# muzishen/RCDMs

Hardware: AMD Instinct MI355X
Metric: story-frames/sec (stage-2 UNet, 50-step DDIM, 512^2) (higher is better)
Workload: dtype f16; 1 GPU; PororoSV stage-2, 512x512, 50-step DDIM, CFG 2.0, batch=1 story x 5 frames per GPU, ctx 85x768, random-init 1276.9M-param UNet3D; stories_per_gpu=1, latent=64, ddim_steps=50, parallelism=story-replicas x1

## Files before the change

rcdms_amd/csrc/rowff.hip:

```cpp
#include "common.h"
#include "pp_sync.h"
#include <type_traits>

#ifndef RCDM_FF_ABLATE
#define RCDM_FF_ABLATE 0
#endif

namespace {

enum { TAIL_FF = 0, TAIL_N1 = 1, TAIL_FFP = 2, TAIL_N3 = 3, TAIL_ATT = 4 };

struct RowArgs {
  const f16* a_in;
  const f16* res;
  f16* tok;
  f16* out;
  const f16* wstream;
  const float* a_bias;
  const float* ln_g;
  const float* ln_b;
  const float* pe;
  const float* b1p;
  const float* b2;
  const f16* z_res;
  const float* z_bias;
  const float* gn_stat;
  const float* gn_g;
  const float* gn_b;
  int M, lda, ldr, ldt, ldo, ldz;
  int rows_per_frame, frames;
  int gn_G, gn_rows;
  float eps;
  float att_scale;
};

template <int C, int NW, int R, int PD, bool HAS_A, bool A_RES, bool LN_PE, int TAIL>
__global__ __launch_bounds__(NW * 64) void row_chain_kernel(const RowArgs p) {
  constexpr int NK = C / 32;
  constexpr int NOF = C / 16;
  constexpr int CHF = 2 * NK;
  constexpr int CHB = CHF * 1024;
  constexpr int NG = C / 8;
  constexpr int NCH_A = HAS_A ? NK : 0;
  constexpr bool IS_FF = TAIL == TAIL_FF || TAIL == TAIL_FFP;
  constexpr bool FM = TAIL == TAIL_ATT;
  constexpr int NCH_T = IS_FF ? 3 * NG + (TAIL == TAIL_FFP ? NK : 0) : (FM ? 3 : TAIL) * NK;
  constexpr int NCH = NCH_A + NCH_T;
  constexpr int NT = NW * 64;
  constexpr int PPW = CHF / NW;
  static_assert(CHF % NW == 0, "chunk fragments must divide over the waves");
  static_assert(NOF == CHF && CHF % PD == 0 && CHF >= 20 && NOF % 2 == 0, "chunk geometry");
  constexpr int PAR0 = R * CHB;
  constexpr int RS = 2 * C + 16;
  static_assert(!IS_FF || NW * 16 * RS <= R * CHB, "epilogue staging exceeds the ring");
  constexpr int XOFF = PAR0 + 3 * C * 4, XW = (NK / 2) * 1024;
  static_assert(!FM || (HAS_A && NW == 10 && (5 * C + NW * 2 * C) * 4 <= NW * XW), "frame-major chain geometry");
  extern __shared__ __attribute__((aligned(16))) char smem[];

  const int t = threadIdx.x, lane = t & 63;
  const int wave = __builtin_amdgcn_readfirstlane(t >> 6);
  const int l15 = lane & 15, kg = lane >> 4;
  int row0_ = blockIdx.x * (NW * 16) + wave * 16, fm_gps = 1, fm_ngrp = 0;
  bool fm_live = true;
  const int fm_f = wave % 5;
  if constexpr (FM) {
    fm_gps = p.rows_per_frame >> 4;
    fm_ngrp = (p.M / (5 * p.rows_per_frame)) * fm_gps;
    const int grp = 2 * blockIdx.x + wave / 5;
    fm_live = grp < fm_ngrp;
    const int g2 = fm_live ? grp : 0, b = g2 / fm_gps;
    row0_ = (b * 5 + fm_f) * p.rows_per_frame + 16 * (g2 - b * fm_gps);
  }
  const int row0 = row0_;
  const int row = row0 + l15;
  const bool live = FM ? fm_live : row < p.M;
  const int oG = HAS_A ? C : 0, oB = oG + C, oPE = oB + C, oT = oPE + (LN_PE ? p.frames * C : 0);
  const int oZ = oT + (IS_FF ? 8 * C : 0);
  const int oGN = oZ + (TAIL == TAIL_FFP ? 2 * C : 0);
  const int npar = oGN;

  const __amdgpu_buffer_rsrc_t rsrcW =
      __builtin_amdgcn_make_buffer_rsrc((void*)p.wstream, 0, (unsigned)NCH * CHB, 0x00020000);
  int dma_voff = lane * 16;
  auto issue_chunk = [&](int c, int slot) __attribute__((always_inline)) {
#pragma unroll
    for (int i = 0; i < PPW; ++i) {
      const int piece = wave * PPW + i;
      const unsigned voff = c < NCH ? (unsigned)dma_voff : 0x80000000u;
      __builtin_amdgcn_raw_ptr_buffer_load_lds(rsrcW, (__attribute__((address_space(3))) void*)(smem + slot * CHB + piece * 1024),
                                               16, voff, c < NCH ? c * CHB + piece * 1024 : 0, 0, 0);
    }
  };

  f16x8 xr[NK];
  f16x8 tk[NK];
  auto ld16 = [](const f16* q) __attribute__((always_inline)) -> f16x8 { Pack16 t; t.u = *(const uint4*)q; return t.h; };
  auto st16 = [](f16* q, f16x8 v) __attribute__((always_inline)) { Pack16 t; t.h = v; *(uint4*)q = t.u; };
  {
    const f16* xp = p.a_in + (size_t)(live ? row : 0) * p.lda + 8 * kg;
#pragma unroll
    for (int s = 0; s < NK; ++s) xr[s] = ld16(xp + 32 * s);
    if (HAS_A && A_RES) {
      const f16* rp = p.res + (size_t)(live ? row : 0) * p.ldr + 8 * kg;
#pragma unroll
      for (int s = 0; s < NK; ++s) tk[s] = ld16(rp + 32 * s);
    } else {
#pragma unroll
      for (int s = 0; s < NK; ++s)
#pragma unroll
        for (int j = 0; j < 8; ++j) tk[s][j] = (f16)0.f;
    }
  }
  constexpr int NB4_MAX = ((HAS_A ? C : 0) + 2 * C + (LN_PE ? 8 * C : 0) + (IS_FF ? 8 * C : 0) + (TAIL == TAIL_FFP ? 2 * C : 0)) / 4;
  constexpr int NB4_PER = (NB4_MAX + NT - 1) / NT;
  f32x4 bq[NB4_PER];
#pragma unroll
  for (int i = 0; i < NB4_PER; ++i) {
    const int idx = min(i * NT + t, npar / 4 - 1) * 4;
    const float* src;
    if (HAS_A && idx < oG) src = p.a_bias + idx;
    else if (idx < oB) src = p.ln_g + (idx - oG);
    else if (idx < oPE) src = p.ln_b + (idx - oB);
    else if (LN_PE && idx < oT) src = p.pe + (idx - oPE);
    else if (idx < oZ) src = p.b1p + (idx - oT);
    else if (idx < oZ + C) src = p.b2 + (idx - oZ);
    else src = p.z_bias + (idx - oZ - C);
    bq[i] = *(const f32x4*)src;
  }
  float gn_sc = 0.f, gn_sh = 0.f;
  float fm_sc[FM ? 5 : 1], fm_sh[FM ? 5 : 1];
  constexpr bool CAN_GN = HAS_A && !A_RES;
  static_assert(NT == 2 * C, "one thread per (sample slot, channel)");
  if constexpr (FM && CAN_GN) {
    if (p.gn_stat) {
      const int j0 = t >= C ? 1 : 0, ch = t - j0 * C;
      const float ga = p.gn_g[ch], be = p.gn_b[ch];
#pragma unroll
      for (int i = 0; i < 5; ++i) {
        const int j = 2 * i + j0;
        const int smp = (min(2 * (int)blockIdx.x + j / 5, fm_ngrp - 1) / fm_gps) * 5 + j % 5;
        const float* st = p.gn_stat + ((size_t)smp * p.gn_G + ch / (C / p.gn_G)) * 2;
        const float mean = st[0], rstd = st[1];
        fm_sc[i] = rstd * ga;
        fm_sh[i] = __builtin_fmaf(-(mean * rstd), ga, be);
      }
// ... 71 lines not shown
  auto run_chunk = [&](auto&& mfma_i, auto&& slice_i, auto&& post_sync) __attribute__((always_inline)) {
    wait_vm<(R - 3) * PPW>();
    if (!(RCDM_FF_ABLATE & 8)) tick_barrier();
    if (!(RCDM_FF_ABLATE & 1)) issue_chunk(c + R - 1, cslot == 0 ? R - 1 : cslot - 1);
    post_sync();
    const char* sb = smem + cslot * CHB + lane16;
    const char* sn = smem + (cslot == R - 1 ? 0 : cslot + 1) * CHB + lane16;
    __builtin_amdgcn_sched_barrier(0);
#pragma unroll
    for (int i = 0; i < CHF; ++i) {
      const f16x8 cur = fr[i % PD];
      mfma_i(i, cur);
      fr[i % PD] = rd(i + PD < CHF ? sb + (i + PD) * 1024 : sn + (i + PD - CHF) * 1024);
      slice_i(i);
      __builtin_amdgcn_sched_barrier(0);
    }
    ++c;
    cslot = cslot == R - 1 ? 0 : cslot + 1;
  };
  auto nothing = [&](int) __attribute__((always_inline)) {};
  auto no_stores = [&]() __attribute__((always_inline)) {};
  const f32x4 z4 = {0.f, 0.f, 0.f, 0.f};

  if constexpr (HAS_A) {
#pragma unroll
    for (int h = 0; h < 2; ++h) {
      f32x4 acc[NOF / 2];
#pragma unroll
      for (int cc = 0; cc < NK / 2; ++cc)
        run_chunk([&](int i, f16x8 w) __attribute__((always_inline)) {
          const int s = 2 * cc + i / (NOF / 2), fi = i % (NOF / 2);
          acc[fi] = mm(w, xr[s], s == 0 ? z4 : acc[fi]);
        }, nothing, no_stores);
#pragma unroll
      for (int fi = 0; fi < NOF / 2; ++fi) {
        const int i = h * (NOF / 2) + fi, s = i >> 1, sub = i & 1;
        const f32x4 b = *(const f32x4*)(par + 32 * s + 8 * kg + 4 * sub);
#pragma unroll
        for (int e = 0; e < 4; ++e) tk[s][4 * sub + e] = (f16)(acc[fi][e] + b[e] + (float)tk[s][4 * sub + e]);
      }
    }
  }
  if (HAS_A && live) {
    f16* tp = p.tok + (size_t)row * p.ldt + 8 * kg;
#pragma unroll
    for (int s = 0; s < NK; ++s) st16(tp + 32 * s, tk[s]);
  }

  {
    f16x8 (&src)[NK] = HAS_A ? tk : xr;
    float s = 0.f;
#pragma unroll
    for (int k = 0; k < NK; ++k)
#pragma unroll
      for (int j = 0; j < 8; ++j) s += (float)src[k][j];
    s += __shfl_xor(s, 16, 64);
    s += __shfl_xor(s, 32, 64);
    const float mean = s * (1.0f / C);
    float q = 0.f;
#pragma unroll
    for (int k = 0; k < NK; ++k)
#pragma unroll
      for (int j = 0; j < 8; ++j) {
        const float d = (float)src[k][j] - mean;
        q += d * d;
      }
    q += __shfl_xor(q, 16, 64);
    q += __shfl_xor(q, 32, 64);
    const float rstd = rsqrtf(q * (1.0f / C) + p.eps);
    const float* pep = !LN_PE ? par : FM ? par + oPE + fm_f * C : par + oPE + (((live ? row : 0) / p.rows_per_frame) % p.frames) * C;
#pragma unroll
    for (int k = 0; k < NK; ++k) {
      const int ch = 32 * k + 8 * kg;
      const f32x4 g0 = *(const f32x4*)(par + oG + ch), g1 = *(const f32x4*)(par + oG + ch + 4);
      f32x4 b0 = *(const f32x4*)(par + oB + ch), b1 = *(const f32x4*)(par + oB + ch + 4);
      if (LN_PE) {
        b0 += *(const f32x4*)(pep + ch);
        b1 += *(const f32x4*)(pep + ch + 4);
      }
      f16x8 y;
#pragma unroll
      for (int j = 0; j < 4; ++j) {
        y[j] = (f16)(((float)src[k][j] - mean) * rstd * g0[j] + b0[j]);
        y[4 + j] = (f16)(((float)src[k][4 + j] - mean) * rstd * g1[j] + b1[j]);
      }
      xr[k] = y;
    }
  }

  auto gemm_groups = [&](auto ngrp_c, auto zadd_c) __attribute__((always_inline)) {
    constexpr int NGRP = decltype(ngrp_c)::value;
    constexpr bool ZADD = decltype(zadd_c)::value;
    f16x8 pend[NOF / 4], zr[ZADD ? NOF / 4 : 1];
    int pend_col = 0;
    auto store_pend = [&]() __attribute__((always_inline)) {
      if (live) {
        f16* op = p.out + (size_t)row * p.ldo + pend_col + 8 * kg;
#pragma unroll
        for (int m = 0; m < NOF / 4; ++m) st16(op + 32 * m, pend[m]);
      }
    };
    for (int grp = 0; grp < NGRP; ++grp) {
      f32x4 acc[NOF / 2];
#pragma unroll
      for (int cc = 0; cc < NK / 2; ++cc) {
        auto mf = [&](int i, f16x8 w) __attribute__((always_inline)) {
          const int s = 2 * cc + i / (NOF / 2), fi = i % (NOF / 2);
          acc[fi] = mm(w, xr[s], s == 0 ? z4 : acc[fi]);
        };
        if (cc == 0)
          run_chunk(mf, nothing, [&]() __attribute__((always_inline)) {
// ... 17 lines not shown
            pend[m][e] = (f16)((float)(f16)(acc[2 * m][e] + b0[e]) + (float)zr[m][e]);
            pend[m][4 + e] = (f16)((float)(f16)(acc[2 * m + 1][e] + b1[e]) + (float)zr[m][4 + e]);
          }
        } else {
#pragma unroll
          for (int e = 0; e < 4; ++e) {
            pend[m][e] = (f16)acc[2 * m][e];
            pend[m][4 + e] = (f16)acc[2 * m + 1][e];
          }
        }
      }
      pend_col = grp * (C / 2);
    }
    wait_lgkm0();
    wait_vm<0>();
    store_pend();
  };

  if constexpr (FM) {
    constexpr int HG = NK / 2;
    char* const X = smem + XOFF;
    const int kgq = lane16 >> 8, xme = wave * XW + lane16, xgrp = (wave / 5) * 5 * XW + lane16;
    const bool c1 = kgq == 0, c2 = kgq <= 1, c3 = kgq <= 2;
    f16x8 qh[HG], pend[HG], oh[HG];
    f32x4 acc[NOF / 2];
    float sc[4][5], o8[8];
    auto round_to = [&](f16x8 (&dst)[HG]) __attribute__((always_inline)) {
#pragma unroll
      for (int m = 0; m < HG; ++m)
#pragma unroll
        for (int e = 0; e < 4; ++e) {
          dst[m][e] = (f16)acc[2 * m][e];
          dst[m][4 + e] = (f16)acc[2 * m + 1][e];
        }
    };
    auto xput = [&]() __attribute__((always_inline)) {
#pragma unroll
      for (int m = 0; m < HG; ++m) *(f16x8*)(X + xme + m * 1024) = pend[m];
    };
    auto xget = [&](int fp, int m) __attribute__((always_inline)) -> f16x8 { return *(const f16x8*)(X + xgrp + fp * XW + m * 1024); };
    auto score_item = [&](int fp, int m) __attribute__((always_inline)) {
      const f16x8 kv = xget(fp, m);
      float d = 0.f;
#pragma unroll
      for (int e = 0; e < 8; e += 2)
        d = __builtin_amdgcn_fdot2(f16x2{qh[m][e], qh[m][e + 1]}, f16x2{kv[e], kv[e + 1]}, d, false);
      if (m == 0) {
// ... 14 lines not shown
      v += __shfl_xor(v, 16, 64);
      v += __shfl_xor(v, 32, 64);
      asm volatile("" : "+v"(v));
      sc[h][fp] = v;
    };
    auto softmax_head = [&](int h) __attribute__((always_inline)) {
      float mx = sc[h][0] * p.att_scale;
#pragma unroll
      for (int j = 0; j < 5; ++j) {
        sc[h][j] *= p.att_scale;
        mx = fmaxf(mx, sc[h][j]);
      }
      float sum = 0.f;
#pragma unroll
      for (int j = 0; j < 5; ++j) {
        sc[h][j] = __expf(sc[h][j] - mx);
        sum += sc[h][j];
      }
      const float inv = __builtin_amdgcn_rcpf(sum);
#pragma unroll
      for (int j = 0; j < 5; ++j) sc[h][j] *= inv;
      asm volatile("" : "+v"(sc[h][0]), "+v"(sc[h][1]), "+v"(sc[h][2]), "+v"(sc[h][3]), "+v"(sc[h][4]));
    };
    auto pv_item = [&](int m, int fp) __attribute__((always_inline)) {
      const f16x8 vv = xget(fp, m);
      const float pj = m == 0 ? sc[0][fp] : m == 4 ? sc[3][fp] : (m == 1 ? c1 : m == 2 ? c2 : c3) ? sc[m - 1][fp] : sc[m][fp];
#pragma unroll
      for (int e = 0; e < 8; ++e) o8[e] = __builtin_fmaf(pj, (float)vv[e], fp == 0 ? 0.f : o8[e]);
      if (fp == 4) {
#pragma unroll
        for (int e = 0; e < 8; ++e) oh[m][e] = (f16)o8[e];
        asm volatile("" : "+v"(oh[m]));
      } else {
        asm volatile("" : "+v"(o8[0]), "+v"(o8[1]), "+v"(o8[2]), "+v"(o8[3]), "+v"(o8[4]), "+v"(o8[5]), "+v"(o8[6]), "+v"(o8[7]));
      }
    };
    auto store_o = [&](int half) __attribute__((always_inline)) {
      if (live) {
        f16* op = p.out + (size_t)row * p.ldo + half * (C / 2) + 8 * kgq;
#pragma unroll
        for (int m = 0; m < HG; ++m) st16(op + 32 * m, oh[m]);
      }
    };
    auto group = [&](auto hh_c, auto grp_c) __attribute__((always_inline)) {
      constexpr int hh = decltype(hh_c)::value, grp = decltype(grp_c)::value;
#pragma unroll
      for (int cc = 0; cc < HG; ++cc)
        run_chunk(
            [&](int i, f16x8 w) __attribute__((always_inline)) {
              const int s = 2 * cc + i / (NOF / 2), fi = i % (NOF / 2);
              acc[fi] = mm(w, xr[s], s == 0 ? z4 : acc[fi]);
            },
            [&](int i) __attribute__((always_inline)) {
              if constexpr (grp == 2) {
                if (cc >= 1 && cc <= 3 && i < (cc == 3 ? 5 : 10)) score_item(2 * (cc - 1) + i / 5, i % 5);
                if (cc == 4) reduce_item(i / 5, i % 5);
              } else if constexpr (grp == 0 && hh == 1) {
                if (cc == 0 && i % 5 == 2) softmax_head(i / 5);
                if (cc >= 1 && cc <= 3 && i < (cc == 3 ? 5 : 10)) pv_item(2 * (cc - 1) + i / 5, i % 5);
              }
            },
            [&]() __attribute__((always_inline)) {
              if (cc == 0 && (grp == 2 || (grp == 0 && hh == 1))) xput();
              if (cc == 0 && grp == 1 && hh == 1) store_o(0);
            });
      if constexpr (grp == 0) round_to(qh); else round_to(pend);
    };
    using I0 = std::integral_constant<int, 0>;
    using I1 = std::integral_constant<int, 1>;
    using I2 = std::integral_constant<int, 2>;
    group(I0{}, I0{}); group(I0{}, I1{}); group(I0{}, I2{});
    group(I1{}, I0{}); group(I1{}, I1{}); group(I1{}, I2{});
#pragma unroll
    for (int h = 0; h < 4; ++h) softmax_head(h);
    wait_lgkm0();
    wait_vm<0>();
    tick_barrier();
    xput();
    wait_lgkm0();
    tick_barrier();
#pragma unroll
    for (int m = 0; m < HG; ++m)
#pragma unroll
      for (int fp = 0; fp < 5; ++fp) pv_item(m, fp);
    store_o(1);
    return;
  } else if constexpr (!IS_FF) {
    gemm_groups(std::integral_constant<int, 2 * TAIL>{}, std::false_type{});
    return;
  } else {
    f32x4 oacc[NOF];
#pragma unroll
    for (int i = 0; i < NOF; ++i) oacc[i] = z4;
    struct GegluState { float bh, x, t, pl, ex; };
    auto geglu_slice = [&](int i, GegluState& st, const f32x4& ah, const f32x4& ag, int gp, f16* dst) __attribute__((always_inline)) {
// ... 182 lines not shown
    const int l15 = L & 15, kg = L >> 4;
    float v;
    if (part < 2) {
      const int s = f >> 1, gate = f & 1;
      const int hr = 32 * g + 16 * part + l15;
      v = w1[(size_t)(gate ? 4 * C + hr : hr) * C + 32 * s + 8 * kg + j];
    } else {
      const int hid = 32 * g + (j < 4 ? 4 * kg + j : 16 + 4 * kg + (j - 4));
      const int n = pperm ? 32 * (f >> 1) + 8 * (l15 >> 2) + 4 * (f & 1) + (l15 & 3) : 16 * f + l15;
      v = w2[(size_t)n * (4 * C) + hid];
    }
    ws[idx] = (f16)v;
    if (idx < (size_t)8 * C) {
      const int q = (int)idx, gp = q >> 5, l = q & 31;
      const int hr = 16 * gp + (l & 15);
      b1p[q] = b1[l < 16 ? hr : 4 * C + hr];
    }
  }
}

template <bool HAS_A, bool A_RES, bool LN_PE, int TAIL>
int launch_chain(const RowArgs& a, hipStream_t stream) {
  constexpr int C = 320, NW = 10, PD = 2;
  constexpr int R = TAIL == TAIL_ATT ? 5 : 7;
  constexpr int CHB = 2 * (C / 32) * 1024;
  const int npar = (HAS_A ? C : 0) + 2 * C + (LN_PE ? a.frames * C : 0) + (TAIL == TAIL_FF || TAIL == TAIL_FFP ? 8 * C : 0) +
                   (TAIL == TAIL_FFP ? 2 * C : 0);
  const int lds = TAIL == TAIL_ATT ? R * CHB + 3 * C * 4 + NW * (C / 64) * 1024 : R * CHB + (npar + (a.gn_stat ? 4 * C : 0)) * 4;
  if (lds > 160 * 1024) return RCDM_ESHAPE;
  static bool attr_set[64] = {};
  if (rcdm_first_on_device(attr_set) &&
      hipFuncSetAttribute((const void*)row_chain_kernel<C, NW, R, PD, HAS_A, A_RES, LN_PE, TAIL>,
                          hipFuncAttributeMaxDynamicSharedMemorySize, 160 * 1024) != hipSuccess)
    return RCDM_ELAUNCH;
  const int nblocks = (a.M + NW * 16 - 1) / (NW * 16);
  hipLaunchKernelGGL((row_chain_kernel<C, NW, R, PD, HAS_A, A_RES, LN_PE, TAIL>), dim3(nblocks), dim3(NW * 64), lds, stream, a);
  return rcdm_check_launch();
}

inline unsigned grid_for(size_t n) {
  size_t g = (n + 255) / 256;
  return (unsigned)(g > 8192 ? 8192 : (g < 1 ? 1 : g));
}

inline bool misaligned16(const void* p) { return p && ((uintptr_t)p & 15); }
inline bool rows_overflow(int M, int ld) { return (size_t)M * (size_t)ld * 2 >= 0x7FFFFFFFull; }

}

extern "C" {

int rcdm_ff_fused_supported(int32_t C) { return C == 320 ? 1 : 0; }
int rcdm_rowchain_supported(int32_t C) { return C == 320 ? 1 : 0; }

int rcdm_rowchain_config_supported(int32_t C, int32_t tail, int32_t pe_frames) {
  if (C != 320 || tail < 0 || tail > 4) return 0;
  if (pe_frames < 0 || pe_frames > 8) return 0;
  if (tail == 4 && pe_frames != 0 && pe_frames != 5) return 0;
  if (pe_frames > 0 && (tail == 0 || tail == 2)) return 0;
  return 1;
}

size_t rcdm_ff_stream_bytes(int32_t C) { return C > 0 ? (size_t)24 * C * C : 0; }

size_t rcdm_rowchain_stream_bytes(int32_t C, int32_t tail) {
  if (C <= 0 || tail < 0 || tail > 4) return 0;
  return (size_t)2 * C * C * (1 + (tail == 0 ? 12 : tail == 2 ? 13 : tail == 4 ? 3 : tail));
}

int rcdm_pack_ff_stream(const float* w1, const float* b1, const float* w2, int32_t C, void* wstream, float* b1_packed,
                        void* stream) {
  if (!w1 || !b1 || !w2 || !wstream || !b1_packed || C <= 0) return RCDM_EINVAL;
  if (C % 32) return RCDM_ESHAPE;
  hipLaunchKernelGGL(pack_ff_stream_kernel, dim3(grid_for((size_t)12 * C * C)), dim3(256), 0, (hipStream_t)stream, w1, b1, w2, C,
                     (f16*)wstream, b1_packed, 0);
  return rcdm_check_launch();
}

int rcdm_pack_rowchain(const float* wa, int32_t C, int32_t tail, const float* wt, const float* w1, const float* b1,
                       const float* w2, void* wstream, float* b1_packed, void* stream) {
  if (!wa || !wstream || C <= 0) return RCDM_EINVAL;
  if (C % 32 || tail < 0 || tail > 4) return RCDM_ESHAPE;
  const bool ff = tail == 0 || tail == 2;
  if ((ff && (!w1 || !b1 || !w2 || !b1_packed)) || (tail != 0 && !wt)) return RCDM_EINVAL;
  f16* ws = (f16*)wstream;
  hipLaunchKernelGGL(pack_pgemm_kernel, dim3(grid_for((size_t)C * C)), dim3(256), 0, (hipStream_t)stream, wa, C, 1, ws, 0);
  ws += (size_t)C * C;
  if (ff) {
    hipLaunchKernelGGL(pack_ff_stream_kernel, dim3(grid_for((size_t)12 * C * C)), dim3(256), 0, (hipStream_t)stream, w1, b1, w2, C,
// ... 8 lines not shown
}

int rcdm_ff_fused(const rcdm_ff_desc* d, const void* x, const float* ln_gamma, const float* ln_beta, const void* wstream,
                  const float* b1_packed, const float* b2, void* out, void* stream) {
  if (!d || !x || !ln_gamma || !ln_beta || !wstream || !b1_packed || !b2 || !out) return RCDM_EINVAL;
  if (d->M <= 0 || d->ldx < d->C || d->ldo < d->C || (d->ldx & 7) || (d->ldo & 7)) return RCDM_EINVAL;
  if (d->C != 320) return RCDM_ESHAPE;
  if (misaligned16(ln_gamma) || misaligned16(ln_beta) || misaligned16(b1_packed) || misaligned16(b2) || misaligned16(x) ||
      misaligned16(out) || misaligned16(wstream))
    return RCDM_EINVAL;
  if (rows_overflow(d->M, d->ldx) || rows_overflow(d->M, d->ldo)) return RCDM_ESHAPE;
  RowArgs a{};
  a.a_in = (const f16*)x; a.out = (f16*)out; a.wstream = (const f16*)wstream;
  a.ln_g = ln_gamma; a.ln_b = ln_beta; a.b1p = b1_packed; a.b2 = b2;
  a.M = d->M; a.lda = d->ldx; a.ldo = d->ldo; a.rows_per_frame = 1; a.frames = 1; a.eps = d->eps;
  return launch_chain<false, false, false, TAIL_FF>(a, (hipStream_t)stream);
}

int rcdm_rowchain(const rcdm_rowchain_desc* d, const void* a_in, const void* res, void* tok, const float* a_bias,
                  const float* ln_gamma, const float* ln_beta, const float* pe, const void* wstream, const float* b1_packed,
                  const float* b2, void* out, const float* gn_stat, const float* gn_gamma, const float* gn_beta,
                  const void* z_res, const float* z_bias, void* stream) {
  if (!d || !a_in || !tok || !a_bias || !ln_gamma || !ln_beta || !wstream || !out) return RCDM_EINVAL;
  const int ncol = d->tail == 0 || d->tail == 2 || d->tail == 4 ? d->C : d->tail * d->C;
  if (d->M <= 0 || d->lda < d->C || d->ldt < d->C || d->ldo < ncol || ((d->lda | d->ldt | d->ldo) & 7)) return RCDM_EINVAL;
  if (res && (d->ldr < d->C || (d->ldr & 7))) return RCDM_EINVAL;
  if (pe && (d->rows_per_frame <= 0 || d->frames <= 0 || d->frames > 8)) return RCDM_EINVAL;
  if ((d->tail == 0 || d->tail == 2) && (!b1_packed || !b2)) return RCDM_EINVAL;
  if (d->C != 320 || d->tail < 0 || d->tail > 4) return RCDM_ESHAPE;
  if (d->tail == 4) {
    if (d->rows_per_frame <= 0 || d->frames <= 0) return RCDM_EINVAL;
    if (d->frames != 5 || d->rows_per_frame % 16 || d->M % (5 * d->rows_per_frame)) return RCDM_ESHAPE;
  }
  if (!rcdm_rowchain_config_supported(d->C, d->tail, pe ? d->frames : 0)) return RCDM_ESHAPE;
  if (misaligned16(a_bias) || misaligned16(ln_gamma) || misaligned16(ln_beta) || misaligned16(pe) || misaligned16(b1_packed) ||
      misaligned16(b2) || misaligned16(z_bias) || misaligned16(gn_gamma) || misaligned16(gn_beta) || misaligned16(a_in) ||
      misaligned16(res) || misaligned16(tok) || misaligned16(out) || misaligned16(z_res) || misaligned16(wstream))
    return RCDM_EINVAL;
  if (rows_overflow(d->M, d->lda) || rows_overflow(d->M, d->ldt) || rows_overflow(d->M, d->ldo) ||
      (res && rows_overflow(d->M, d->ldr)) || (z_res && rows_overflow(d->M, d->ldz)))
    return RCDM_ESHAPE;
  if (d->tail == 2) {
    if (!res || pe || !z_res || !z_bias || d->ldz < d->C || (d->ldz & 7)) return RCDM_EINVAL;
  }
  if (gn_stat) {
    if (res || !gn_gamma || !gn_beta || d->gn_groups <= 0 || d->gn_rows <= 0) return RCDM_EINVAL;
    if (d->C % d->gn_groups || d->gn_rows % 16) return RCDM_ESHAPE;
    if (d->tail == 4 ? d->gn_rows != d->rows_per_frame : d->gn_rows < 160) return RCDM_ESHAPE;
  }
  RowArgs a{};
  a.a_in = (const f16*)a_in; a.res = (const f16*)res; a.tok = (f16*)tok; a.out = (f16*)out; a.wstream = (const f16*)wstream;
  a.a_bias = a_bias; a.ln_g = ln_gamma; a.ln_b = ln_beta; a.pe = pe; a.b1p = b1_packed; a.b2 = b2;
  a.M = d->M; a.lda = d->lda; a.ldr = d->ldr; a.ldt = d->ldt; a.ldo = d->ldo;
  a.rows_per_frame = pe || d->tail == 4 ? d->rows_per_frame : 1; a.frames = pe || d->tail == 4 ? d->frames : 1; a.eps = d->eps;
  a.att_scale = (float)(1.0 / sqrt((double)(d->C / 8)));
  a.z_res = (const f16*)z_res; a.z_bias = z_bias; a.ldz = d->ldz;
  a.gn_stat = gn_stat; a.gn_g = gn_gamma; a.gn_b = gn_beta; a.gn_G = d->gn_groups; a.gn_rows = d->gn_rows;
  hipStream_t s = (hipStream_t)stream;
#define RCDM_CHAIN(T)                                                                  \
  (res ? (pe ? launch_chain<true, true, true, T>(a, s) : launch_chain<true, true, false, T>(a, s)) \
       : (pe ? launch_chain<true, false, true, T>(a, s) : launch_chain<true, false, false, T>(a, s)))
  switch (d->tail) {
    case 0: return RCDM_CHAIN(TAIL_FF);
    case 1: return RCDM_CHAIN(TAIL_N1);
    case 2: return launch_chain<true, true, false, TAIL_FFP>(a, s);
    case 3: return RCDM_CHAIN(TAIL_N3);
    default: return RCDM_CHAIN(TAIL_ATT);
  }
#undef RCDM_CHAIN
}

}
```

rcdms_amd/emit_blocks.py:

```python
import torch

from . import hip
from . import switches as SW
from .emit_ops import (XATTN_MAX_KEYS, assert_no_pending_gn, conv3x3_wino_ok, emit_conv3x3, emit_conv3x3_wino, emit_flash_attn, emit_gemm,
                       emit_groupnorm, emit_groupnorm_stats, emit_layernorm, emit_temporal_attn, emit_xattn, emit_xattn_pack, gemm_lnx_ok)
from .packer import MSUB_SCORE_LIMIT, attn_score_bound
from .plan import Rows, _NS


def emit_resnet(plan, w, x, geo, temb, out, eps=1e-5, groups=32, out_scale=1.0, dup_rows=0, out_gn=None):
    g = geo
    u1, u2 = getattr(w, "wino1", None) is not None, getattr(w, "wino2", None) is not None
    rv = (temb[0], temb[1], temb[2], g.f * g.hw)
    cross = (g.b, g.f * g.hw, groups)
    assert not (u1 or u2) or (not dup_rows and x.C == w.cin)
    h1 = plan.rows("res_h1", g.M, w.cout)
    res = x

    def unfolded_shortcut():
        if u2 or w.shortcut is None:
            return x
        sc = plan.rows("res_sc", g.M, w.cout)
        emit_gemm(plan, x, w.shortcut, w.cout, w.cin, sc, bias=w.sb)
        return sc
# ... 307 lines not shown
    return r1


def emit_motion(plan, w, x, geo, heads, out, groups=32, prior_state=False, out_gn=None):
    g, C = geo, w.C
    d_head = C // heads
    a = plan.rows("norm", g.M, C)
    chained = (w.chains is not None and not prior_state and g.M >= CHAIN_MIN_ROWS and
               hip.rowchain_config_supported(C, 3, g.f))
    gn = None
    if prior_state:
        emit_layernorm(plan, x, w.prior_g, w.prior_b, a)
    elif chained and g.hw % 16 == 0 and g.hw >= 160:
        gn = emit_groupnorm_stats(plan, x, g.n_img, g.hw, w.gn_g, w.gn_b, 1e-6, groups)
    else:
        emit_groupnorm(plan, x, g.n_img, g.hw, w.gn_g, w.gn_b, 1e-6, False, a, groups)
    z, tok = (None, plan.rows("tok", g.M, C)) if chained else ffz_rows(plan, w, g.M, C, x, out)
    if chained:
        qkv = plan.rows("qkv", g.M, 3 * C)
        ao = plan.rows("attn_out", g.M, C)
        a0, a1 = w.attn
        if (w.chains_att is not None and g.f == 5 and heads == 8 and g.hw % 16 == 0 and g.M >= MOTION_FUSE_MIN_ROWS and
                hip.rowchain_config_supported(C, 4, g.f)):
            emit_rowchain(plan, x if gn else a, None, tok, w.proj_in_b, (a0.ln_g, a0.ln_b), a0.pe, w.chains_att[0], 4, ao, g.hw, g.f, gn=gn)
            emit_rowchain(plan, ao, tok, tok, a0.o_b, (a1.ln_g, a1.ln_b), a1.pe, w.chains_att[1], 4, ao, g.hw, g.f)
        else:
            emit_rowchain(plan, x if gn else a, None, tok, w.proj_in_b, (a0.ln_g, a0.ln_b), a0.pe, w.chains[0], 3, qkv, g.hw, g.f, gn=gn)
            emit_temporal_attn(plan, qkv, g.b, g.f, g.hw, heads, d_head, ao)
            emit_rowchain(plan, ao, tok, tok, a0.o_b, (a1.ln_g, a1.ln_b), a1.pe, w.chains[1], 3, qkv, g.hw, g.f)
            emit_temporal_attn(plan, qkv, g.b, g.f, g.hw, heads, d_head, ao)
        if w.chain_ffz is not None:
            emit_rowchain(plan, ao, tok, tok, a1.o_b, w.ff_ln, None, w.chain_ffz, 2, out, b2=w.ff2_b, z=(x, w.proj_out_b))
            return
        emit_rowchain(plan, ao, tok, tok, a1.o_b, w.ff_ln, None, w.chains[2], 0, tok, b2=w.ff2_b)
        emit_gemm(plan, tok, w.proj_out, C, C, out, bias=w.proj_out_b, residual=x)
        return
    want_stat = SW.LNX and g.M < CHAIN_MIN_ROWS
    st = emit_gemm(plan, a, w.proj_in, C, C, tok, bias=w.proj_in_b, stat=want_stat)
    for at in w.attn:
        qkv = plan.rows("qkv", g.M, 3 * C)
        lx = at.lnx
        if st is not None and lx is not None and gemm_lnx_ok(g.M, 3 * C, C, tok.ld, qkv.ld) and (at.pe is None or g.f <= at.pe.shape[0]):
            if at.pe is not None:
                tab = lx.tab[:g.f].repeat(g.b, 1).contiguous()
                emit_gemm(plan, tok, lx.W, 3 * C, C, qkv, rowvec=(tab, 0, 3 * C, g.hw), lnx=(st, lx.S))
            else:
                emit_gemm(plan, tok, lx.W, 3 * C, C, qkv, bias=lx.b, lnx=(st, lx.S))
        else:
# ... 10 lines not shown
```

rcdms_amd/packer.py:

```python
import math

import torch

from . import hip
from . import switches as SW
from .plan import _NS


class Packer:
    def __init__(self, sd, device):
        self.sd, self.device = sd, torch.device(device)
        self._tmp = []

    def f32(self, key):
        t = self.sd[key].detach().to(self.device, torch.float32).contiguous()
        return t

    def has(self, key):
        return key in self.sd

    def vec(self, key):
        return self.f32(key)

    def mat_f16(self, *keys):
# ... 122 lines not shown
            wz = self.f32(wt_keys[0])
            if w1.shape != (8 * Cc, Cc) or w2.shape != (Cc, 4 * Cc) or wz.numel() != Cc * Cc:
                return None
            wz = wz.reshape(Cc, Cc).contiguous()
            b1p = torch.empty(8 * Cc, dtype=torch.float32, device=self.device)
            hip.pack_rowchain(wa.data_ptr(), Cc, 2, wz.data_ptr(), w1.data_ptr(), b1.data_ptr(), w2.data_ptr(), ws.data_ptr(),
                              b1p.data_ptr())
            self._tmp += [wa, wz, w1, b1, w2]
            return ws, b1p
        if tail:
            wt = torch.cat([self.f32(k) for k in wt_keys], dim=0).contiguous()
            if tuple(wt.shape) != ((3 if tail == 4 else tail) * Cc, Cc):
                return None
            hip.pack_rowchain(wa.data_ptr(), Cc, tail, wt.data_ptr(), 0, 0, 0, ws.data_ptr(), 0)
            self._tmp += [wa, wt]
            return ws, None
        w1, b1, w2 = (self.f32(k) for k in ff_keys)
        if w1.shape != (8 * Cc, Cc) or w2.shape != (Cc, 4 * Cc):
            return None
        b1p = torch.empty(8 * Cc, dtype=torch.float32, device=self.device)
        hip.pack_rowchain(wa.data_ptr(), Cc, 0, 0, w1.data_ptr(), b1.data_ptr(), w2.data_ptr(), ws.data_ptr(), b1p.data_ptr())
        self._tmp += [wa, w1, b1, w2]
        return ws, b1p

    def done(self):
        torch.cuda.synchronize(self.device)
        self._tmp.clear()


def pack_resnet(pk, p, wino=(False, False)):
    w = _NS(cin=pk.sd[p + "conv1.weight"].shape[1], cout=pk.sd[p + "conv1.weight"].shape[0])
    w.g1, w.b1 = pk.vec(p + "norm1.weight"), pk.vec(p + "norm1.bias")
    w.g2, w.b2 = pk.vec(p + "norm2.weight"), pk.vec(p + "norm2.bias")
    u1, u2 = (bool(wino), bool(wino)) if isinstance(wino, bool) else wino
    w.wino1 = w.wino2 = None
    if u1:
        w.wino1, w.cb1, w.conv1 = pk.conv3x3_wino(p + "conv1.weight"), pk.vec(p + "conv1.bias"), None
    if u2:
        w.wino2, w.cb2 = pk.conv3x3_wino(p + "conv2.weight"), pk.vec(p + "conv2.bias")
        w.conv2 = w.shortcut = w.conv2sc = None
        if pk.has(p + "conv_shortcut.weight"):
            w.shortcut, w.sb = pk.mat_f16(p + "conv_shortcut.weight"), pk.vec(p + "conv_shortcut.bias")
            w.cb2sc = (w.cb2 + w.sb).contiguous()
    if not u1:
        w.conv1, w.cb1 = pk.conv3x3(p + "conv1.weight"), pk.vec(p + "conv1.bias")
    if u2:
# ... 103 lines not shown
    b = p + "transformer_blocks.0."
    w = _NS(C=C)
    w.gn_g, w.gn_b = pk.vec(p + "norm.weight"), pk.vec(p + "norm.bias")
    if pk.has(p + "prior_norm.weight"):
        w.prior_g, w.prior_b = pk.vec(p + "prior_norm.weight"), pk.vec(p + "prior_norm.bias")
    w.proj_in, w.proj_in_b = pk.mat_f16(p + "proj_in.weight"), pk.vec(p + "proj_in.bias")
    w.proj_out, w.proj_out_b = pk.mat_f16(p + "proj_out.weight"), pk.vec(p + "proj_out.bias")
    w.attn = []
    for i in range(n_attn):
        a = b + f"attention_blocks.{i}."
        pe = pk.f32(a + "pos_encoder.pe")[0].contiguous() if pk.has(a + "pos_encoder.pe") else None
        ln_g, ln_b = pk.vec(b + f"norms.{i}.weight"), pk.vec(b + f"norms.{i}.bias")
        w.attn.append(_NS(
            ln_g=ln_g, ln_b=ln_b, pe=pe,
            qkv=pk.mat_f16(a + "to_q.weight", a + "to_k.weight", a + "to_v.weight"),
            lnx=pk.lnx_mat((a + "to_q.weight", a + "to_k.weight", a + "to_v.weight"), ln_g, ln_b, pe=pe) if lnx else None,
            o=pk.mat_f16(a + "to_out.0.weight"), o_b=pk.vec(a + "to_out.0.bias")))
    w.ff_ln = (pk.vec(b + "ff_norm.weight"), pk.vec(b + "ff_norm.bias"))
    w.lnx_ff = pk.lnx_geglu(b + "ff.net.0.proj.weight", b + "ff.net.0.proj.bias", *w.ff_ln) if lnx else None
    w.ff1, w.ff1_b = pk.geglu(b + "ff.net.0.proj.weight", b + "ff.net.0.proj.bias")
    w.ff2, w.ff2_b = pk.mat_f16(b + "ff.net.2.weight"), pk.vec(b + "ff.net.2.bias")
    w.ff_stream = pk.ff_stream(b + "ff.net.0.proj.weight", b + "ff.net.0.proj.bias", b + "ff.net.2.weight")
    w.ffz = pk.ffz(b + "ff.net.2.weight", b + "ff.net.2.bias", p + "proj_out.weight", p + "proj_out.bias") if lnx else None
    w.chains = w.chain_ffz = w.chains_att = None
    if n_attn == 2:
        a0, a1 = b + "attention_blocks.0.", b + "attention_blocks.1."
        qkv = lambda a: (a + "to_q.weight", a + "to_k.weight", a + "to_v.weight")
        ch = [pk.chain(p + "proj_in.weight", 3, wt_keys=qkv(a0)), pk.chain(a0 + "to_out.0.weight", 3, wt_keys=qkv(a1)),
              pk.chain(a1 + "to_out.0.weight", 0,
                       ff_keys=(b + "ff.net.0.proj.weight", b + "ff.net.0.proj.bias", b + "ff.net.2.weight"))]
        if all(c is not None for c in ch) and all(at.pe is not None for at in w.attn):
            w.chains = ch
            if SW.MOTION_FUSE and hip.rowchain_config_supported(C, 4, 5):
                w.chains_att = [pk.chain(p + "proj_in.weight", 4, wt_keys=qkv(a0)), pk.chain(a0 + "to_out.0.weight", 4, wt_keys=qkv(a1))]
            w.chain_ffz = pk.chain(a1 + "to_out.0.weight", 2, wt_keys=(p + "proj_out.weight",),
                                   ff_keys=(b + "ff.net.0.proj.weight", b + "ff.net.0.proj.bias", b + "ff.net.2.weight"))
    return w
```

rcdms_amd/switches.py:

```python
import os


def _on(name, default="1"):
    return os.environ.get(name, default) != "0"


SC_FOLD = _on("RCDM_SC_FOLD")
UP2 = _on("RCDM_UP2")
GN_PRESTAT = _on("RCDM_GN_PRESTAT")
LNX = _on("RCDM_LNX")
FFZ = _on("RCDM_FFZ")
FF_FUSE = _on("RCDM_FF_FUSE")
ROW_CHAIN = _on("RCDM_ROWCHAIN")
MOTION_FUSE = _on("RCDM_MOTION_FUSE")
RANK1_CTX = _on("RCDM_RANK1_CTX")
_w = os.environ.get("RCDM_WINO", "le32").strip()
WINO_MAX_SIDE = int(_w[2:]) if _w.startswith("le") else 0
WINO_MIN_SIDE = 8
WINO_MIN_C = int(os.environ.get("RCDM_WINO_MIN_C", "640"))
WINO = tuple(int(v) for v in _w.split(",") if v.strip().isdigit() and int(v) > 0) if not _w.startswith("le") else ()


def wino_side(H, W):
    if H % 2 or W % 2:
        return False
    return (min(H, W) >= WINO_MIN_SIDE and max(H, W) <= WINO_MAX_SIDE) if WINO_MAX_SIDE else (H == W and H in WINO)


UP9 = _on("RCDM_UP9")
OUT_TAPS = _on("RCDM_OUT_TAPS")
_vf = os.environ.get("RCDM_VAE_FLASH", "auto").strip().lower()
VAE_FLASH = _vf if _vf in ("0", "1") else "auto"
CHAIN_MIN_ROWS = os.environ.get("RCDM_CHAIN_MIN_ROWS")

TABLE = {
    "RCDM_SC_FOLD": SC_FOLD, "RCDM_UP2": UP2, "RCDM_GN_PRESTAT": GN_PRESTAT, "RCDM_LNX": LNX, "RCDM_FFZ": FFZ,
    "RCDM_FF_FUSE": FF_FUSE, "RCDM_ROWCHAIN": ROW_CHAIN, "RCDM_MOTION_FUSE": MOTION_FUSE, "RCDM_RANK1_CTX": RANK1_CTX, "RCDM_WINO": _w, "RCDM_WINO_MIN_C": WINO_MIN_C, "RCDM_UP9": UP9, "RCDM_OUT_TAPS": OUT_TAPS, "RCDM_CHAIN_MIN_ROWS": CHAIN_MIN_ROWS,
# ... 3 lines not shown
```

Baseline: 5.818 story-frames/s.

## Fuse both motion-module attention blocks into one frame-major row-chain kernel

Adds a TAIL_ATT2 variant of the row-chain kernel that runs two back-to-back motion-attention blocks in a single launch. The second block's to_out projection, residual reload, layer norm and QKV/attention reuse the on-chip state from the first pass, and the weight stream is concatenated. This removes one kernel launch per motion module and the second pass's reload of activations from global memory. In exchange it adds register pressure and more LDS parameter space, and the merged schedule depends on an interleaved softmax/PV overlap. It is enabled by default through MOTION_FUSE=2.

```diff
diff --git a/rcdms_amd/csrc/rowff.hip b/rcdms_amd/csrc/rowff.hip
--- a/rcdms_amd/csrc/rowff.hip
+++ b/rcdms_amd/csrc/rowff.hip
@@ -8,7 +8,7 @@
 
 namespace {
 
-enum { TAIL_FF = 0, TAIL_N1 = 1, TAIL_FFP = 2, TAIL_N3 = 3, TAIL_ATT = 4 };
+enum { TAIL_FF = 0, TAIL_N1 = 1, TAIL_FFP = 2, TAIL_N3 = 3, TAIL_ATT = 4, TAIL_ATT2 = 5 };
 
 struct RowArgs {
   const f16* a_in;
@@ -43,9 +43,10 @@
   constexpr int NG = C / 8;
   constexpr int NCH_A = HAS_A ? NK : 0;
   constexpr bool IS_FF = TAIL == TAIL_FF || TAIL == TAIL_FFP;
-  constexpr bool FM = TAIL == TAIL_ATT;
+  constexpr bool FM = TAIL == TAIL_ATT || TAIL == TAIL_ATT2;
+  constexpr int NPASS = TAIL == TAIL_ATT2 ? 2 : 1;
   constexpr int NCH_T = IS_FF ? 3 * NG + (TAIL == TAIL_FFP ? NK : 0) : (FM ? 3 : TAIL) * NK;
-  constexpr int NCH = NCH_A + NCH_T;
+  constexpr int NCH = NPASS * (NCH_A + NCH_T);
   constexpr int NT = NW * 64;
   constexpr int PPW = CHF / NW;
   static_assert(CHF % NW == 0, "chunk fragments must divide over the waves");
@@ -53,7 +54,7 @@
   constexpr int PAR0 = R * CHB;
   constexpr int RS = 2 * C + 16;
   static_assert(!IS_FF || NW * 16 * RS <= R * CHB, "epilogue staging exceeds the ring");
-  constexpr int XOFF = PAR0 + 3 * C * 4, XW = (NK / 2) * 1024;
+  constexpr int XOFF = PAR0 + NPASS * 3 * C * 4, XW = (NK / 2) * 1024;
   static_assert(!FM || (HAS_A && NW == 10 && (5 * C + NW * 2 * C) * 4 <= NW * XW), "frame-major chain geometry");
   extern __shared__ __attribute__((aligned(16))) char smem[];
 
@@ -74,7 +75,7 @@
   const int row0 = row0_;
   const int row = row0 + l15;
   const bool live = FM ? fm_live : row < p.M;
-  const int oG = HAS_A ? C : 0, oB = oG + C, oPE = oB + C, oT = oPE + (LN_PE ? p.frames * C : 0);
+  const int oG = HAS_A ? C : 0, oB = oG + C, oPE = oB + C + (NPASS - 1) * 3 * C, oT = oPE + (LN_PE ? p.frames * C : 0);
   const int oZ = oT + (IS_FF ? 8 * C : 0);
   const int oGN = oZ + (TAIL == TAIL_FFP ? 2 * C : 0);
   const int npar = oGN;
@@ -111,7 +112,7 @@
         for (int j = 0; j < 8; ++j) tk[s][j] = (f16)0.f;
     }
   }
-  constexpr int NB4_MAX = ((HAS_A ? C : 0) + 2 * C + (LN_PE ? 8 * C : 0) + (IS_FF ? 8 * C : 0) + (TAIL == TAIL_FFP ? 2 * C : 0)) / 4;
+  constexpr int NB4_MAX = ((HAS_A ? C : 0) + 2 * C + (NPASS - 1) * 3 * C + (LN_PE ? 8 * C : 0) + (IS_FF ? 8 * C : 0) + (TAIL == TAIL_FFP ? 2 * C : 0)) / 4;
   constexpr int NB4_PER = (NB4_MAX + NT - 1) / NT;
   f32x4 bq[NB4_PER];
 #pragma unroll
@@ -120,7 +121,10 @@
     const float* src;
     if (HAS_A && idx < oG) src = p.a_bias + idx;
     else if (idx < oB) src = p.ln_g + (idx - oG);
-    else if (idx < oPE) src = p.ln_b + (idx - oB);
+    else if (idx < oB + C) src = p.ln_b + (idx - oB);
+    else if (NPASS == 2 && idx < 4 * C) src = p.a_bias + (idx - 2 * C);
+    else if (NPASS == 2 && idx < 5 * C) src = p.ln_g + (idx - 3 * C);
+    else if (NPASS == 2 && idx < 6 * C) src = p.ln_b + (idx - 4 * C);
     else if (LN_PE && idx < oT) src = p.pe + (idx - oPE);
     else if (idx < oZ) src = p.b1p + (idx - oT);
     else if (idx < oZ + C) src = p.b2 + (idx - oZ);
@@ -238,7 +242,7 @@
   auto no_stores = [&]() __attribute__((always_inline)) {};
   const f32x4 z4 = {0.f, 0.f, 0.f, 0.f};
 
-  if constexpr (HAS_A) {
+  auto stage_a = [&](f16x8 (&opnd)[NK], const float* bias, auto&& slice, auto&& post) __attribute__((always_inline)) {
 #pragma unroll
     for (int h = 0; h < 2; ++h) {
       f32x4 acc[NOF / 2];
@@ -246,24 +250,34 @@
       for (int cc = 0; cc < NK / 2; ++cc)
         run_chunk([&](int i, f16x8 w) __attribute__((always_inline)) {
           const int s = 2 * cc + i / (NOF / 2), fi = i % (NOF / 2);
-          acc[fi] = mm(w, xr[s], s == 0 ? z4 : acc[fi]);
-        }, nothing, no_stores);
+          acc[fi] = mm(w, opnd[s], s == 0 ? z4 : acc[fi]);
+        }, [&](int i) __attribute__((always_inline)) { slice(h, cc, i); }, [&]() __attribute__((always_inline)) { post(h, cc); });
 #pragma unroll
       for (int fi = 0; fi < NOF / 2; ++fi) {
         const int i = h * (NOF / 2) + fi, s = i >> 1, sub = i & 1;
-        const f32x4 b = *(const f32x4*)(par + 32 * s + 8 * kg + 4 * sub);
+        const f32x4 b = *(const f32x4*)(bias + 32 * s + 8 * kg + 4 * sub);
 #pragma unroll
         for (int e = 0; e < 4; ++e) tk[s][4 * sub + e] = (f16)(acc[fi][e] + b[e] + (float)tk[s][4 * sub + e]);
       }
-    }
-  }
-  if (HAS_A && live) {
-    f16* tp = p.tok + (size_t)row * p.ldt + 8 * kg;
-#pragma unroll
-    for (int s = 0; s < NK; ++s) st16(tp + 32 * s, tk[s]);
-  }
-
-  {
+      if constexpr (NPASS == 2) {
+#pragma unroll
+        for (int s = h * (NK / 2); s < (h + 1) * (NK / 2); ++s) asm volatile("" : "+v"(tk[s]));
+      }
+    }
+  };
+  auto store_tok = [&]() __attribute__((always_inline)) {
+    if (live) {
+      f16* tp = p.tok + (size_t)row * p.ldt + 8 * kg;
+#pragma unroll
+      for (int s = 0; s < NK; ++s) st16(tp + 32 * s, tk[s]);
+    }
+  };
+  if constexpr (HAS_A) {
+    stage_a(xr, par, [&](int, int, int) __attribute__((always_inline)) {}, [&](int, int) __attribute__((always_inline)) {});
+    store_tok();
+  }
+
+  auto layer_norm = [&](const float* pg) __attribute__((always_inline)) {
     f16x8 (&src)[NK] = HAS_A ? tk : xr;
     float s = 0.f;
 #pragma unroll
@@ -284,12 +298,14 @@
     q += __shfl_xor(q, 16, 64);
     q += __shfl_xor(q, 32, 64);
     const float rstd = rsqrtf(q * (1.0f / C) + p.eps);
+    int kgl = NPASS == 2 ? lane16 >> 8 : kg;
+    if (NPASS == 2) asm volatile("" : "+v"(kgl));
     const float* pep = !LN_PE ? par : FM ? par + oPE + fm_f * C : par + oPE + (((live ? row : 0) / p.rows_per_frame) % p.frames) * C;
 #pragma unroll
     for (int k = 0; k < NK; ++k) {
-      const int ch = 32 * k + 8 * kg;
-      const f32x4 g0 = *(const f32x4*)(par + oG + ch), g1 = *(const f32x4*)(par + oG + ch + 4);
-      f32x4 b0 = *(const f32x4*)(par + oB + ch), b1 = *(const f32x4*)(par + oB + ch + 4);
+      const int ch = 32 * k + 8 * kgl;
+      const f32x4 g0 = *(const f32x4*)(pg + oG + ch), g1 = *(const f32x4*)(pg + oG + ch + 4);
+      f32x4 b0 = *(const f32x4*)(pg + oB + ch), b1 = *(const f32x4*)(pg + oB + ch + 4);
       if (LN_PE) {
         b0 += *(const f32x4*)(pep + ch);
         b1 += *(const f32x4*)(pep + ch + 4);
@@ -302,7 +318,8 @@
       }
       xr[k] = y;
     }
-  }
+  };
+  layer_norm(par);
 
   auto gemm_groups = [&](auto ngrp_c, auto zadd_c) __attribute__((always_inline)) {
     constexpr int NGRP = decltype(ngrp_c)::value;
@@ -366,7 +383,7 @@
     char* const X = smem + XOFF;
     const int kgq = lane16 >> 8, xme = wave * XW + lane16, xgrp = (wave / 5) * 5 * XW + lane16;
     const bool c1 = kgq == 0, c2 = kgq <= 1, c3 = kgq <= 2;
-    f16x8 qh[HG], pend[HG], oh[HG];
+    f16x8 qh[HG], pend[HG], oh[NPASS == 2 ? NK : HG];
     f32x4 acc[NOF / 2];
     float sc[4][5], o8[8];
     auto round_to = [&](f16x8 (&dst)[HG]) __attribute__((always_inline)) {
@@ -427,15 +444,15 @@
       for (int j = 0; j < 5; ++j) sc[h][j] *= inv;
       asm volatile("" : "+v"(sc[h][0]), "+v"(sc[h][1]), "+v"(sc[h][2]), "+v"(sc[h][3]), "+v"(sc[h][4]));
     };
-    auto pv_item = [&](int m, int fp) __attribute__((always_inline)) {
+    auto pv_item = [&](int m, int fp, int ob = 0) __attribute__((always_inline)) {
       const f16x8 vv = xget(fp, m);
       const float pj = m == 0 ? sc[0][fp] : m == 4 ? sc[3][fp] : (m == 1 ? c1 : m == 2 ? c2 : c3) ? sc[m - 1][fp] : sc[m][fp];
 #pragma unroll
       for (int e = 0; e < 8; ++e) o8[e] = __builtin_fmaf(pj, (float)vv[e], fp == 0 ? 0.f : o8[e]);
       if (fp == 4) {
 #pragma unroll
-        for (int e = 0; e < 8; ++e) oh[m][e] = (f16)o8[e];
-        asm volatile("" : "+v"(oh[m]));
+        for (int e = 0; e < 8; ++e) oh[ob + m][e] = (f16)o8[e];
+        asm volatile("" : "+v"(oh[ob + m]));
       } else {
         asm volatile("" : "+v"(o8[0]), "+v"(o8[1]), "+v"(o8[2]), "+v"(o8[3]), "+v"(o8[4]), "+v"(o8[5]), "+v"(o8[6]), "+v"(o8[7]));
       }
@@ -447,8 +464,9 @@
         for (int m = 0; m < HG; ++m) st16(op + 32 * m, oh[m]);
       }
     };
-    auto group = [&](auto hh_c, auto grp_c) __attribute__((always_inline)) {
+    auto group = [&](auto last_c, auto hh_c, auto grp_c) __attribute__((always_inline)) {
       constexpr int hh = decltype(hh_c)::value, grp = decltype(grp_c)::value;
+      constexpr bool last = decltype(last_c)::value;
 #pragma unroll
       for (int cc = 0; cc < HG; ++cc)
         run_chunk(
@@ -467,15 +485,59 @@
             },
             [&]() __attribute__((always_inline)) {
               if (cc == 0 && (grp == 2 || (grp == 0 && hh == 1))) xput();
-              if (cc == 0 && grp == 1 && hh == 1) store_o(0);
+              if (cc == 0 && grp == 1 && hh == 1 && last) store_o(0);
             });
       if constexpr (grp == 0) round_to(qh); else round_to(pend);
     };
     using I0 = std::integral_constant<int, 0>;
     using I1 = std::integral_constant<int, 1>;
     using I2 = std::integral_constant<int, 2>;
-    group(I0{}, I0{}); group(I0{}, I1{}); group(I0{}, I2{});
-    group(I1{}, I0{}); group(I1{}, I1{}); group(I1{}, I2{});
+    auto groups = [&](auto last_c) __attribute__((always_inline)) {
+      group(last_c, I0{}, I0{}); group(last_c, I0{}, I1{}); group(last_c, I0{}, I2{});
+      group(last_c, I1{}, I0{}); group(last_c, I1{}, I1{}); group(last_c, I1{}, I2{});
+    };
+    groups(std::integral_constant<bool, NPASS == 1>{});
+    if constexpr (NPASS == 2) {
+      const __amdgpu_buffer_rsrc_t rsrcT = __builtin_amdgcn_make_buffer_rsrc((void*)p.tok, 0, 0x7FFFFFFF, 0x00020000);
+      const int t_e = wave * 64 + (lane16 >> 4), peq = min(t_e, 5 * C / 4 - 1);
+      f32x4 pe1 = z4;
+      stage_a(oh, par + 3 * C,
+              [&](int h, int cc, int i) __attribute__((always_inline)) {
+                if (h == 0 && cc == 0 && i % 5 == 2) softmax_head(i / 5);
+                if (h == 0 && cc >= 1 && cc <= 3 && i < (cc == 3 ? 5 : 10)) pv_item(2 * (cc - 1) + i / 5, i % 5, HG);
+              },
+              [&](int h, int cc) __attribute__((always_inline)) {
+                if (h == 0 && cc == 0) xput();
+                if (cc == 3) {
+                  int off = ((live ? row : 0) * p.ldt + 8 * (lane16 >> 8)) * 2 + h * C;
+                  asm volatile("" : "+v"(off));
+#pragma unroll
+                  for (int s = 0; s < HG; ++s) {
+                    Pack16 tt;
+                    tt.v = __builtin_amdgcn_raw_buffer_load_b128(rsrcT, off + 64 * s, 0, 16);
+                    tk[h * HG + s] = tt.h;
+                  }
+                }
+                if (LN_PE && h == 1 && cc == 0) {
+                  int pq = 4 * peq;
+                  asm volatile("" : "+v"(pq));
+                  pe1 = *(const f32x4*)(p.pe + 5 * C + pq);
+                }
+                if (LN_PE && h == 1 && cc == 2) *(f32x4*)(X + 16 * t_e) = pe1;
+              });
+      if (live) {
+        int off = (row * p.ldt + 8 * (lane16 >> 8)) * 2;
+        asm volatile("" : "+v"(off));
+#pragma unroll
+        for (int s = 0; s < NK; ++s) {
+          Pack16 tt;
+          tt.h = tk[s];
+          __builtin_amdgcn_raw_buffer_store_b128(tt.v, rsrcT, off + 64 * s, 0, 0);
+        }
+      }
+      layer_norm(par + 3 * C);
+      groups(std::true_type{});
+    }
 #pragma unroll
     for (int h = 0; h < 4; ++h) softmax_head(h);
     wait_lgkm0();
@@ -704,11 +766,12 @@
 template <bool HAS_A, bool A_RES, bool LN_PE, int TAIL>
 int launch_chain(const RowArgs& a, hipStream_t stream) {
   constexpr int C = 320, NW = 10, PD = 2;
-  constexpr int R = TAIL == TAIL_ATT ? 5 : 7;
+  constexpr bool ATT = TAIL == TAIL_ATT || TAIL == TAIL_ATT2;
+  constexpr int R = ATT ? 5 : 7;
   constexpr int CHB = 2 * (C / 32) * 1024;
   const int npar = (HAS_A ? C : 0) + 2 * C + (LN_PE ? a.frames * C : 0) + (TAIL == TAIL_FF || TAIL == TAIL_FFP ? 8 * C : 0) +
                    (TAIL == TAIL_FFP ? 2 * C : 0);
-  const int lds = TAIL == TAIL_ATT ? R * CHB + 3 * C * 4 + NW * (C / 64) * 1024 : R * CHB + (npar + (a.gn_stat ? 4 * C : 0)) * 4;
+  const int lds = ATT ? R * CHB + (TAIL == TAIL_ATT2 ? 6 : 3) * C * 4 + NW * (C / 64) * 1024 : R * CHB + (npar + (a.gn_stat ? 4 * C : 0)) * 4;
   if (lds > 160 * 1024) return RCDM_ESHAPE;
   static bool attr_set[64] = {};
   if (rcdm_first_on_device(attr_set) &&
@@ -736,9 +799,9 @@
 int rcdm_rowchain_supported(int32_t C) { return C == 320 ? 1 : 0; }
 
 int rcdm_rowchain_config_supported(int32_t C, int32_t tail, int32_t pe_frames) {
-  if (C != 320 || tail < 0 || tail > 4) return 0;
+  if (C != 320 || tail < 0 || tail > 5) return 0;
   if (pe_frames < 0 || pe_frames > 8) return 0;
-  if (tail == 4 && pe_frames != 0 && pe_frames != 5) return 0;
+  if (tail >= 4 && pe_frames != 0 && pe_frames != 5) return 0;
   if (pe_frames > 0 && (tail == 0 || tail == 2)) return 0;
   return 1;
 }
@@ -746,7 +809,8 @@
 size_t rcdm_ff_stream_bytes(int32_t C) { return C > 0 ? (size_t)24 * C * C : 0; }
 
 size_t rcdm_rowchain_stream_bytes(int32_t C, int32_t tail) {
-  if (C <= 0 || tail < 0 || tail > 4) return 0;
+  if (C <= 0 || tail < 0 || tail > 5) return 0;
+  if (tail == 5) return (size_t)2 * 2 * C * C * 4;
   return (size_t)2 * C * C * (1 + (tail == 0 ? 12 : tail == 2 ? 13 : tail == 4 ? 3 : tail));
 }
 
@@ -801,13 +865,13 @@
                   const float* b2, void* out, const float* gn_stat, const float* gn_gamma, const float* gn_beta,
                   const void* z_res, const float* z_bias, void* stream) {
   if (!d || !a_in || !tok || !a_bias || !ln_gamma || !ln_beta || !wstream || !out) return RCDM_EINVAL;
-  const int ncol = d->tail == 0 || d->tail == 2 || d->tail == 4 ? d->C : d->tail * d->C;
+  const int ncol = d->tail == 0 || d->tail == 2 || d->tail >= 4 ? d->C : d->tail * d->C;
   if (d->M <= 0 || d->lda < d->C || d->ldt < d->C || d->ldo < ncol || ((d->lda | d->ldt | d->ldo) & 7)) return RCDM_EINVAL;
   if (res && (d->ldr < d->C || (d->ldr & 7))) return RCDM_EINVAL;
   if (pe && (d->rows_per_frame <= 0 || d->frames <= 0 || d->frames > 8)) return RCDM_EINVAL;
   if ((d->tail == 0 || d->tail == 2) && (!b1_packed || !b2)) return RCDM_EINVAL;
-  if (d->C != 320 || d->tail < 0 || d->tail > 4) return RCDM_ESHAPE;
-  if (d->tail == 4) {
+  if (d->C != 320 || d->tail < 0 || d->tail > 5) return RCDM_ESHAPE;
+  if (d->tail >= 4) {
     if (d->rows_per_frame <= 0 || d->frames <= 0) return RCDM_EINVAL;
     if (d->frames != 5 || d->rows_per_frame % 16 || d->M % (5 * d->rows_per_frame)) return RCDM_ESHAPE;
   }
@@ -819,19 +883,20 @@
   if (rows_overflow(d->M, d->lda) || rows_overflow(d->M, d->ldt) || rows_overflow(d->M, d->ldo) ||
       (res && rows_overflow(d->M, d->ldr)) || (z_res && rows_overflow(d->M, d->ldz)))
     return RCDM_ESHAPE;
+  if (d->tail == 5 && res) return RCDM_EINVAL;
   if (d->tail == 2) {
     if (!res || pe || !z_res || !z_bias || d->ldz < d->C || (d->ldz & 7)) return RCDM_EINVAL;
   }
   if (gn_stat) {
     if (res || !gn_gamma || !gn_beta || d->gn_groups <= 0 || d->gn_rows <= 0) return RCDM_EINVAL;
     if (d->C % d->gn_groups || d->gn_rows % 16) return RCDM_ESHAPE;
-    if (d->tail == 4 ? d->gn_rows != d->rows_per_frame : d->gn_rows < 160) return RCDM_ESHAPE;
+    if (d->tail >= 4 ? d->gn_rows != d->rows_per_frame : d->gn_rows < 160) return RCDM_ESHAPE;
   }
   RowArgs a{};
   a.a_in = (const f16*)a_in; a.res = (const f16*)res; a.tok = (f16*)tok; a.out = (f16*)out; a.wstream = (const f16*)wstream;
   a.a_bias = a_bias; a.ln_g = ln_gamma; a.ln_b = ln_beta; a.pe = pe; a.b1p = b1_packed; a.b2 = b2;
   a.M = d->M; a.lda = d->lda; a.ldr = d->ldr; a.ldt = d->ldt; a.ldo = d->ldo;
-  a.rows_per_frame = pe || d->tail == 4 ? d->rows_per_frame : 1; a.frames = pe || d->tail == 4 ? d->frames : 1; a.eps = d->eps;
+  a.rows_per_frame = pe || d->tail >= 4 ? d->rows_per_frame : 1; a.frames = pe || d->tail >= 4 ? d->frames : 1; a.eps = d->eps;
   a.att_scale = (float)(1.0 / sqrt((double)(d->C / 8)));
   a.z_res = (const f16*)z_res; a.z_bias = z_bias; a.ldz = d->ldz;
   a.gn_stat = gn_stat; a.gn_g = gn_gamma; a.gn_b = gn_beta; a.gn_G = d->gn_groups; a.gn_rows = d->gn_rows;
@@ -844,7 +909,8 @@
     case 1: return RCDM_CHAIN(TAIL_N1);
     case 2: return launch_chain<true, true, false, TAIL_FFP>(a, s);
     case 3: return RCDM_CHAIN(TAIL_N3);
-    default: return RCDM_CHAIN(TAIL_ATT);
+    case 4: return RCDM_CHAIN(TAIL_ATT);
+    default: return pe ? launch_chain<true, false, true, TAIL_ATT2>(a, s) : launch_chain<true, false, false, TAIL_ATT2>(a, s);
   }
 #undef RCDM_CHAIN
 }
diff --git a/rcdms_amd/emit_blocks.py b/rcdms_amd/emit_blocks.py
--- a/rcdms_amd/emit_blocks.py
+++ b/rcdms_amd/emit_blocks.py
@@ -353,8 +353,12 @@
         a0, a1 = w.attn
         if (w.chains_att is not None and g.f == 5 and heads == 8 and g.hw % 16 == 0 and g.M >= MOTION_FUSE_MIN_ROWS and
                 hip.rowchain_config_supported(C, 4, g.f)):
-            emit_rowchain(plan, x if gn else a, None, tok, w.proj_in_b, (a0.ln_g, a0.ln_b), a0.pe, w.chains_att[0], 4, ao, g.hw, g.f, gn=gn)
-            emit_rowchain(plan, ao, tok, tok, a0.o_b, (a1.ln_g, a1.ln_b), a1.pe, w.chains_att[1], 4, ao, g.hw, g.f)
+            if w.chain_att2 is not None and hip.rowchain_config_supported(C, 5, g.f):
+                a_b, ln2, pe2 = w.att2_par
+                emit_rowchain(plan, x if gn else a, None, tok, a_b, ln2, pe2, w.chain_att2, 5, ao, g.hw, g.f, gn=gn)
+            else:
+                emit_rowchain(plan, x if gn else a, None, tok, w.proj_in_b, (a0.ln_g, a0.ln_b), a0.pe, w.chains_att[0], 4, ao, g.hw, g.f, gn=gn)
+                emit_rowchain(plan, ao, tok, tok, a0.o_b, (a1.ln_g, a1.ln_b), a1.pe, w.chains_att[1], 4, ao, g.hw, g.f)
         else:
             emit_rowchain(plan, x if gn else a, None, tok, w.proj_in_b, (a0.ln_g, a0.ln_b), a0.pe, w.chains[0], 3, qkv, g.hw, g.f, gn=gn)
             emit_temporal_attn(plan, qkv, g.b, g.f, g.hw, heads, d_head, ao)
diff --git a/rcdms_amd/packer.py b/rcdms_amd/packer.py
--- a/rcdms_amd/packer.py
+++ b/rcdms_amd/packer.py
@@ -168,6 +168,14 @@
         hip.pack_rowchain(wa.data_ptr(), Cc, 0, 0, w1.data_ptr(), b1.data_ptr(), w2.data_ptr(), ws.data_ptr(), b1p.data_ptr())
         self._tmp += [wa, w1, b1, w2]
         return ws, b1p
+
+    def chain_att2(self, wa_keys, wt_keys):
+        parts = [self.chain(wa, 4, wt_keys=wt) for wa, wt in zip(wa_keys, wt_keys)]
+        if any(c is None for c in parts):
+            return None
+        ws = torch.cat([c[0] for c in parts])
+        assert ws.numel() == hip.rowchain_stream_bytes(self.sd[wa_keys[0]].shape[0], 5)
+        return ws, None
 
     def done(self):
         torch.cuda.synchronize(self.device)
@@ -317,7 +325,7 @@
     w.ff2, w.ff2_b = pk.mat_f16(b + "ff.net.2.weight"), pk.vec(b + "ff.net.2.bias")
     w.ff_stream = pk.ff_stream(b + "ff.net.0.proj.weight", b + "ff.net.0.proj.bias", b + "ff.net.2.weight")
     w.ffz = pk.ffz(b + "ff.net.2.weight", b + "ff.net.2.bias", p + "proj_out.weight", p + "proj_out.bias") if lnx else None
-    w.chains = w.chain_ffz = w.chains_att = None
+    w.chains = w.chain_ffz = w.chains_att = w.chain_att2 = None
     if n_attn == 2:
         a0, a1 = b + "attention_blocks.0.", b + "attention_blocks.1."
         qkv = lambda a: (a + "to_q.weight", a + "to_k.weight", a + "to_v.weight")
@@ -328,6 +336,12 @@
             w.chains = ch
             if SW.MOTION_FUSE and hip.rowchain_config_supported(C, 4, 5):
                 w.chains_att = [pk.chain(p + "proj_in.weight", 4, wt_keys=qkv(a0)), pk.chain(a0 + "to_out.0.weight", 4, wt_keys=qkv(a1))]
+            if SW.MOTION_FUSE >= 2 and hip.rowchain_config_supported(C, 5, 5) and all(at.pe.shape[0] >= 5 for at in w.attn):
+                w.chain_att2 = pk.chain_att2((p + "proj_in.weight", a0 + "to_out.0.weight"), (qkv(a0), qkv(a1)))
+                at0, at1 = w.attn
+                w.att2_par = (torch.stack([w.proj_in_b, at0.o_b]).contiguous(),
+                              (torch.stack([at0.ln_g, at1.ln_g]).contiguous(), torch.stack([at0.ln_b, at1.ln_b]).contiguous()),
+                              torch.stack([at0.pe[:5], at1.pe[:5]]).contiguous())
             w.chain_ffz = pk.chain(a1 + "to_out.0.weight", 2, wt_keys=(p + "proj_out.weight",),
                                    ff_keys=(b + "ff.net.0.proj.weight", b + "ff.net.0.proj.bias", b + "ff.net.2.weight"))
     return w
diff --git a/rcdms_amd/switches.py b/rcdms_amd/switches.py
--- a/rcdms_amd/switches.py
+++ b/rcdms_amd/switches.py
@@ -12,7 +12,8 @@
 FFZ = _on("RCDM_FFZ")
 FF_FUSE = _on("RCDM_FF_FUSE")
 ROW_CHAIN = _on("RCDM_ROWCHAIN")
-MOTION_FUSE = _on("RCDM_MOTION_FUSE")
+_mf = os.environ.get("RCDM_MOTION_FUSE", "2").strip()
+MOTION_FUSE = int(_mf) if _mf.isdigit() else 2
 RANK1_CTX = _on("RCDM_RANK1_CTX")
 _w = os.environ.get("RCDM_WINO", "le32").strip()
 WINO_MAX_SIDE = int(_w[2:]) if _w.startswith("le") else 0
```

Result: no change. 5.838 story-frames/s (median of 6 runs) (+0.3%).
